# deepinv/deepinv

Hardware: AMD Instinct MI355X
Metric: PnP-PGD slices/sec (50 iters), 2D MRI 8-coil 320x320, 4x radial mask, DRUNet (higher is better)
Workload: dtype f32: fp32 multiplies and accumulation on the fp32 matrix cores (v_mfma_f32_32x32x2_f32); ResBlock convs as Winograd F(4x4,3x3), U = G g G^T formed in fp64 and rounded once; the three 2x2 stride-2 down convolutions (2 % of the FLOPs) as an exact three-part bf16 operand split with six products and fp3

## Files before the change

### deepinv_amd/csrc/drunet_bf16s.hip

```cpp
#include "drunet_common.hpp"

using namespace dinv;
using namespace dinv_drunet;

namespace {

__device__ __forceinline__ unsigned f2bf(float f) {
#ifdef DINV_EMU
    unsigned u = __float_as_uint(f);
    if ((u & 0x7fffffffu) > 0x7f800000u) return (u >> 16) | 0x40u;
    u += 0x7fffu + ((u >> 16) & 1u);
    return u >> 16;
#else
    return (unsigned)__builtin_bit_cast(unsigned short, (__bf16)f);
#endif
}
__device__ __forceinline__ float bf2f(unsigned h) { return __uint_as_float(h << 16); }

__device__ __forceinline__ void split8(const float4& a, const float4& b, uint4& hi, uint4& lo) {
    const float v[8] = {a.x, a.y, a.z, a.w, b.x, b.y, b.z, b.w};
    unsigned h[8], l[8];
#pragma unroll
    for (int e = 0; e < 8; ++e) {
        h[e] = f2bf(v[e]);
        l[e] = f2bf(v[e] - bf2f(h[e]));
    }
    hi = make_uint4(h[0] | (h[1] << 16), h[2] | (h[3] << 16), h[4] | (h[5] << 16), h[6] | (h[7] << 16));
    lo = make_uint4(l[0] | (l[1] << 16), l[2] | (l[3] << 16), l[4] | (l[5] << 16), l[6] | (l[7] << 16));
}

__device__ __forceinline__ void split8x3(const float4& a, const float4& b, uint4& hi, uint4& mi, uint4& lo) {
    const float v[8] = {a.x, a.y, a.z, a.w, b.x, b.y, b.z, b.w};
    unsigned h[8], m[8], l[8];
#pragma unroll
    for (int e = 0; e < 8; ++e) {
        h[e] = f2bf(v[e]);
        const float r1 = v[e] - bf2f(h[e]);
        m[e] = f2bf(r1);
        l[e] = f2bf(r1 - bf2f(m[e]));
    }
    hi = make_uint4(h[0] | (h[1] << 16), h[2] | (h[3] << 16), h[4] | (h[5] << 16), h[6] | (h[7] << 16));
    mi = make_uint4(m[0] | (m[1] << 16), m[2] | (m[3] << 16), m[4] | (m[5] << 16), m[6] | (m[7] << 16));
    lo = make_uint4(l[0] | (l[1] << 16), l[2] | (l[3] << 16), l[4] | (l[5] << 16), l[6] | (l[7] << 16));
}

#ifdef DINV_EMU
__device__ __forceinline__ f32x16 mfma_bf16(const uint4& a, const uint4& b, const f32x16& c) {
    emu_bf16x8 av, bv;
    std::memcpy(&av, &a, 16);
    std::memcpy(&bv, &b, 16);
    return emu_mfma_f32_32x32x16_bf16(av, bv, c);
}
#else
typedef __bf16 bf16x8 __attribute__((ext_vector_type(8)));
__device__ __forceinline__ f32x16 mfma_bf16(const uint4& a, const uint4& b, const f32x16& c) {
    return __builtin_amdgcn_mfma_f32_32x32x16_bf16(__builtin_bit_cast(bf16x8, a), __builtin_bit_cast(bf16x8, b), c, 0, 0, 0);
}
#endif

struct DownSArgs {
    Geom gi, go;
    const float* x;
    const uint4* w;
    float* y;
    int32_t cin, cout;
    int64_t ntiles, per_xcd;
    DepthMap dm;
};

template <bool ACC, int NPL>
__global__ __launch_bounds__(256) void down2x2_bf16s_kernel(DownSArgs a) {
    constexpr int WU = NPL * 128;
    constexpr int WPT = (WU + 255) / 256;
    __shared__ uint4 wl[2][WU];
    const int tid = threadIdx.x, lane = tid & 63, wv = tid >> 6;
    const int l31 = lane & 31, lhi = lane >> 5;
    const int64_t logical = (int64_t)(blockIdx.x & 7) * a.per_xcd + (blockIdx.x >> 3);
    if (logical >= a.ntiles) return;
    const int nct = a.cout / 64;
    const int64_t q0 = (logical / nct) * 256 + wv * 64;
    const int co0 = (int)(logical % nct) * 64;
    int64_t ioff[2];
    bool in[2];
#pragma unroll
    for (int n = 0; n < 2; ++n) {
        const int64_t q = q0 + n * 32 + l31;
        in[n] = interior(a.go, q);
        ioff[n] = a.gi.sl;
        if (in[n]) {
            const int64_t b = q / a.go.plane;
            const int64_t bi = depth_pair(a.dm, b);
            if (bi < 0) in[n] = false;
            else {
                const int qi = (int)(q - b * a.go.plane);
                const int R = qi / a.go.wp, C = qi - R * a.go.wp;
                ioff[n] = a.gi.sl + bi * a.gi.plane + (int64_t)(2 * (R - 1) + 1) * a.gi.wp + (2 * (C - 1) + 1);
            }
        }
    }
    f32x16 acc[2][2];
#pragma unroll
    for (int m = 0; m < 2; ++m)
#pragma unroll
        for (int n = 0; n < 2; ++n)
#pragma unroll
            for (int r = 0; r < 16; ++r) acc[m][n][r] = 0.f;
    const int S = a.cin / 16, nsteps = 4 * S;
    float4 ba[2], bb[2];
    uint4 wreg[WPT];
    auto issue = [&](int g) {
        const int tap = g / S, s = g - tap * S;
        const int64_t toff = (int64_t)(tap >> 1) * a.gi.wp + (tap & 1);
#pragma unroll
        for (int k = 0; k < WPT; ++k) {
            const int u = tid + 256 * k;
            if (u < WU) wreg[k] = a.w[((int64_t)g * (2 * NPL) + (u >> 6)) * a.cout + co0 + (u & 63)];
        }
#pragma unroll
        for (int n = 0; n < 2; ++n) {
            const float* xb = a.x + ((int64_t)(2 * s + lhi) * a.gi.cs + ioff[n] + toff) * 8;
            ba[n] = ld4(xb);
            bb[n] = ld4(xb + 4);
        }
    };
    uint4 Bp[NPL][2];
    auto commit = [&](int stage) {
#pragma unroll
        for (int k = 0; k < WPT; ++k)
            if (tid + 256 * k < WU) wl[stage][tid + 256 * k] = wreg[k];
#pragma unroll
        for (int n = 0; n < 2; ++n) {
            if constexpr (NPL == 2) split8(ba[n], bb[n], Bp[0][n], Bp[1][n]);
            else split8x3(ba[n], bb[n], Bp[0][n], Bp[1][n], Bp[2][n]);
        }
    };
    issue(0);
    commit(0);
    if (nsteps > 1) issue(1);
    __syncthreads();
    constexpr int NPROD = NPL == 2 ? 3 : 6;
    constexpr int PA[6] = {0, 1, 0, 0, 1, 0}, PB2[3] = {1, 0, 0};
    constexpr int QA[6] = {1, 0, 2, 0, 1, 0}, QB[6] = {1, 2, 0, 1, 0, 0};
    for (int g = 0; g < nsteps; ++g) {
        const uint4* ws = wl[g & 1];
        uint4 A[NPL][2];
#pragma unroll
        for (int pl = 0; pl < NPL; ++pl)
#pragma unroll
            for (int m = 0; m < 2; ++m) A[pl][m] = ws[pl * 128 + lhi * 64 + m * 32 + l31];
#pragma unroll
        for (int e = 0; e < NPROD; ++e) {
            const int pa = NPL == 2 ? PA[e] : QA[e], pb = NPL == 2 ? PB2[e] : QB[e];
#pragma unroll
            for (int m = 0; m < 2; ++m)
#pragma unroll
                for (int n = 0; n < 2; ++n) acc[m][n] = mfma_bf16(A[pa][m], Bp[pb][n], acc[m][n]);
        }
        if (g + 1 < nsteps) {
            commit((g + 1) & 1);
            if (g + 2 < nsteps) issue(g + 2);
        }
        lds_barrier();
    }
#pragma unroll
    for (int n = 0; n < 2; ++n) {
        const int64_t q = q0 + n * 32 + l31;
        if (q >= a.go.np) continue;
        store_tile<2, false, ACC ? 1 : 0>(acc, n, a.go.sl + q, in[n], co0 / 8, a.cout / 8, a.go.cs, lhi, a.y, ACC ? a.y : nullptr,
                                          nullptr);
    }
}

struct UpSArgs {
    Geom gi, go;
    const float* x;
    const float* x2;
    const uint4* w;
    float* y;
    int32_t cin, cout;
    DepthMap dm;
};

#ifdef DINV_EMU
#define DINV_BF16S_UP_ATTR
#else
#define DINV_BF16S_UP_ATTR __attribute__((amdgpu_waves_per_eu(2, 2)))
#endif
template <bool SKIP>
__global__ __launch_bounds__(256) DINV_BF16S_UP_ATTR void up2x2_bf16s_kernel(UpSArgs a) {
    __shared__ uint4 wl[2][1024];
    const int tid = threadIdx.x, lane = tid & 63, wv = tid >> 6;
    const int l31 = lane & 31, lhi = lane >> 5;
    const int tp = wv & 1, pg = wv >> 1;
    const int co0 = blockIdx.y * 64;
    const int64_t p0 = (int64_t)blockIdx.x * 128 + pg * 64;
    int64_t ioff[2], ooff[2];
    bool in[2];
#pragma unroll
    for (int n = 0; n < 2; ++n) {
        const int64_t p = p0 + n * 32 + l31;
        in[n] = interior(a.gi, p);
        ioff[n] = a.gi.sl + (in[n] ? p : 0);
        ooff[n] = 0;
        if (in[n]) {
            const int64_t b = p / a.gi.plane;
            const int64_t bo = depth_pair(a.dm, b);
            if (bo < 0) in[n] = false;
            else {
                const int pi = (int)(p - b * a.gi.plane);
                const int r = pi / a.gi.wp, c = pi - r * a.gi.wp;
                ooff[n] = a.go.sl + bo * a.go.plane + (int64_t)(2 * (r - 1) + 1 + tp) * a.go.wp + (2 * (c - 1) + 1);
            }
        }
    }
    f32x16 acc[2][2][2];
#pragma unroll
    for (int t = 0; t < 2; ++t)
#pragma unroll
        for (int m = 0; m < 2; ++m)
#pragma unroll
            for (int n = 0; n < 2; ++n)
#pragma unroll
                for (int r = 0; r < 16; ++r) acc[t][m][n][r] = 0.f;
    const int S = a.cin / 16;
    float4 ba[2], bb[2];
    uint4 wreg[4];
    auto issue = [&](int s) {
#pragma unroll
        for (int k = 0; k < 4; ++k) {
            const int u = tid + 256 * k;
            wreg[k] = a.w[((int64_t)s * 16 + (u >> 6)) * a.cout + co0 + (u & 63)];
        }
#pragma unroll
        for (int n = 0; n < 2; ++n) {
            const int64_t o = ((int64_t)(2 * s + lhi) * a.gi.cs + ioff[n]) * 8;
            ba[n] = ld4(a.x + o);
            bb[n] = ld4(a.x + o + 4);
            if (SKIP) {
                ba[n] = add4(ba[n], ld4(a.x2 + o));
                bb[n] = add4(bb[n], ld4(a.x2 + o + 4));
            }
        }
    };
    auto commit = [&](int stage, uint4 (&Bh)[2], uint4 (&Bl)[2]) {
#pragma unroll
        for (int k = 0; k < 4; ++k) wl[stage][tid + 256 * k] = wreg[k];
        split8(ba[0], bb[0], Bh[0], Bl[0]);
        split8(ba[1], bb[1], Bh[1], Bl[1]);
    };
    uint4 Bh[2], Bl[2];
    issue(0);
    commit(0, Bh, Bl);
    if (S > 1) issue(1);
    __syncthreads();
    for (int s = 0; s < S; ++s) {
        const uint4* ws = wl[s & 1] + (tp * 2) * 256;
#pragma unroll
        for (int t = 0; t < 2; ++t) {
            uint4 A[2][2];
#pragma unroll
            for (int pl = 0; pl < 2; ++pl)
#pragma unroll
                for (int m = 0; m < 2; ++m) A[pl][m] = ws[t * 256 + pl * 128 + lhi * 64 + m * 32 + l31];
#pragma unroll
            for (int e = 0; e < 3; ++e) {
                const int pa = e == 1 ? 1 : 0;
#pragma unroll
                for (int m = 0; m < 2; ++m)
#pragma unroll
                    for (int n = 0; n < 2; ++n) acc[t][m][n] = mfma_bf16(A[pa][m], e == 0 ? Bl[n] : Bh[n], acc[t][m][n]);
            }
        }
        if (s + 1 < S) {
            commit((s + 1) & 1, Bh, Bl);
            if (s + 2 < S) issue(s + 2);
        }
        lds_barrier();
    }
#pragma unroll
    for (int n = 0; n < 2; ++n) {
        if (!in[n]) continue;
#pragma unroll
        for (int t = 0; t < 2; ++t)
#pragma unroll
            for (int m = 0; m < 2; ++m)
#pragma unroll
                for (int rj = 0; rj < 4; ++rj) {
                    const float4 v = make_float4(acc[t][m][n][4 * rj], acc[t][m][n][4 * rj + 1], acc[t][m][n][4 * rj + 2],
                                                 acc[t][m][n][4 * rj + 3]);
                    st4(a.y + ((int64_t)(co0 / 8 + m * 4 + rj) * a.go.cs + ooff[n] + t) * 8 + 4 * lhi, v);
                }
    }
}

}

static int down2x2_bf16s_launch(const dinv_act_geom* gin, const dinv_act_geom* gout, const float* x, const void* w_split,
                                int32_t cin, int32_t cout, float* y, DepthMap dm, int accumulate, dinv_stream_t stream,
                                int planes = 2) {
    if (int e = check_geom(gin)) return e;
    if (int e = check_geom(gout)) return e;
    DINV_REQUIRE(x && w_split && y, "null tensor pointer");
    DINV_REQUIRE(gin->height == 2 * gout->height && gin->width == 2 * gout->width, "down2x2 geometry mismatch");
    if (dm.dep_s == 0) DINV_REQUIRE(gin->batch == gout->batch, "down2x2 geometry mismatch");
    else
        DINV_REQUIRE(dm.dep_s >= 3 && dm.dep_l == 2 * (dm.dep_s - 2) + 2 && gout->batch % dm.dep_s == 0 &&
                     gin->batch / dm.dep_l == gout->batch / dm.dep_s && gin->batch % dm.dep_l == 0 && (dm.dz == 0 || dm.dz == 1),
                     "down2x2: bad depth pairing (%d, %d, %d)", dm.dep_s, dm.dep_l, dm.dz);
    DINV_REQUIRE(cin >= 16 && cin % 16 == 0 && cout % 64 == 0, "bf16-split down2x2 needs cin %% 16 == 0 and cout %% 64 == 0 (got %d,%d)", cin, cout);
    DownSArgs a{make_geom(*gin), make_geom(*gout), x, reinterpret_cast<const uint4*>(w_split), y, cin, cout, 0, 0, dm};
    a.ntiles = ceil_div(gout->np, 256) * (cout / 64);
    a.per_xcd = ceil_div(a.ntiles, 8);
    const dim3 grid((unsigned)(a.per_xcd * 8));
    hipStream_t st = reinterpret_cast<hipStream_t>(stream);
    if (planes == 3) hipLaunchKernelGGL((down2x2_bf16s_kernel<false, 3>), grid, dim3(256), 0, st, a);
    else if (accumulate) hipLaunchKernelGGL((down2x2_bf16s_kernel<true, 2>), grid, dim3(256), 0, st, a);
    else hipLaunchKernelGGL((down2x2_bf16s_kernel<false, 2>), grid, dim3(256), 0, st, a);
    DINV_CHECK_LAUNCH();
    return 0;
}

extern "C" int dinv_conv_down2x2_bf16s(const dinv_act_geom* gin, const dinv_act_geom* gout, const float* x,
                                       const void* w_split, int32_t cin, int32_t cout, float* y, dinv_stream_t stream) {
    return down2x2_bf16s_launch(gin, gout, x, w_split, cin, cout, y, DepthMap{0, 0, 0}, 0, stream);
}

extern "C" int dinv_conv_down2x2_bf16x3(const dinv_act_geom* gin, const dinv_act_geom* gout, const float* x,
                                        const void* w_split3, int32_t cin, int32_t cout, float* y, dinv_stream_t stream) {
    return down2x2_bf16s_launch(gin, gout, x, w_split3, cin, cout, y, DepthMap{0, 0, 0}, 0, stream, 3);
}

extern "C" int dinv_conv_down2x2_bf16s_3d(const dinv_act_geom* gin, const dinv_act_geom* gout, const float* x,
                                          const void* w_split, int32_t cin, int32_t cout, float* y, int32_t depth_out,
                                          int32_t dz, int32_t accumulate, dinv_stream_t stream) {
    DINV_REQUIRE(depth_out >= 1, "bad depth %d", depth_out);
    return down2x2_bf16s_launch(gin, gout, x, w_split, cin, cout, y, DepthMap{depth_out + 2, 2 * depth_out + 2, dz}, accumulate, stream);
}

static int up2x2_bf16s_launch(const dinv_act_geom* gin, const dinv_act_geom* gout, const float* x, const float* x2,
                              const void* w_split, int32_t cin, int32_t cout, float* y, DepthMap dm, dinv_stream_t stream) {
    if (int e = check_geom(gin)) return e;
    if (int e = check_geom(gout)) return e;
    DINV_REQUIRE(x && w_split && y, "null tensor pointer");
    DINV_REQUIRE(gout->height == 2 * gin->height && gout->width == 2 * gin->width, "up2x2 geometry mismatch");
    if (dm.dep_s == 0) DINV_REQUIRE(gin->batch == gout->batch, "up2x2 geometry mismatch");
    else
        DINV_REQUIRE(dm.dep_s >= 3 && dm.dep_l == 2 * (dm.dep_s - 2) + 2 && gin->batch % dm.dep_s == 0 &&
                     gout->batch % dm.dep_l == 0 && gout->batch / dm.dep_l == gin->batch / dm.dep_s && (dm.dz == 0 || dm.dz == 1),
                     "up2x2: bad depth pairing (%d, %d, %d)", dm.dep_s, dm.dep_l, dm.dz);
    DINV_REQUIRE(cin >= 16 && cin % 16 == 0 && cout % 64 == 0, "bf16-split up2x2 needs cin %% 16 == 0 and cout %% 64 == 0 (got %d,%d)", cin, cout);
    UpSArgs a{make_geom(*gin), make_geom(*gout), x, x2, reinterpret_cast<const uint4*>(w_split), y, cin, cout, dm};
    const dim3 grid((unsigned)ceil_div(gin->np, 128), (unsigned)(cout / 64));
    hipStream_t st = reinterpret_cast<hipStream_t>(stream);
    if (x2) hipLaunchKernelGGL(up2x2_bf16s_kernel<true>, grid, dim3(256), 0, st, a);
    else hipLaunchKernelGGL(up2x2_bf16s_kernel<false>, grid, dim3(256), 0, st, a);
    DINV_CHECK_LAUNCH();
    return 0;
}

extern "C" int dinv_conv_up2x2_bf16s(const dinv_act_geom* gin, const dinv_act_geom* gout, const float* x, const float* x2,
                                     const void* w_split, int32_t cin, int32_t cout, float* y, dinv_stream_t stream) {
    return up2x2_bf16s_launch(gin, gout, x, x2, w_split, cin, cout, y, DepthMap{0, 0, 0}, stream);
}

extern "C" int dinv_conv_up2x2_bf16s_3d(const dinv_act_geom* gin, const dinv_act_geom* gout, const float* x, const float* x2,
                                        const void* w_split, int32_t cin, int32_t cout, float* y, int32_t depth_in, int32_t dz,
                                        dinv_stream_t stream) {
    DINV_REQUIRE(depth_in >= 1, "bad depth %d", depth_in);
    return up2x2_bf16s_launch(gin, gout, x, x2, w_split, cin, cout, y, DepthMap{depth_in + 2, 2 * depth_in + 2, dz}, stream);
}
```

Baseline: 16.22.

## Double-register pipeline and reorder K loop in bf16-split down conv

Rewrites the down2x2 bf16-split kernel's main loop. It now keeps two register sets of prefetched activations and weights and issues the next global load before the MFMAs, unrolling by two. The K iteration is reordered to row-tap-major with pairs of horizontal taps merged into a single channel block (via lhi), which changes the weight packing index. It aims to hide global load latency better at the cost of more registers, and it relies on a matching weight layout on the host side.

Measured after the change: 16.32 (median of 6 runs). Within noise of the previous version (+0.6%).

```diff
diff --git a/deepinv_amd/csrc/drunet_bf16s.hip b/deepinv_amd/csrc/drunet_bf16s.hip
--- a/deepinv_amd/csrc/drunet_bf16s.hip
+++ b/deepinv_amd/csrc/drunet_bf16s.hip
@@ -71,7 +71,6 @@
 template <bool ACC, int NPL>
 __global__ __launch_bounds__(256) void down2x2_bf16s_kernel(DownSArgs a) {
     constexpr int WU = NPL * 128;
-    constexpr int WPT = (WU + 255) / 256;
     __shared__ uint4 wl[2][WU];
     const int tid = threadIdx.x, lane = tid & 63, wv = tid >> 6;
     const int l31 = lane & 31, lhi = lane >> 5;
@@ -105,44 +104,38 @@
         for (int n = 0; n < 2; ++n)
 #pragma unroll
             for (int r = 0; r < 16; ++r) acc[m][n][r] = 0.f;
-    const int S = a.cin / 16, nsteps = 4 * S;
-    float4 ba[2], bb[2];
-    uint4 wreg[WPT];
-    auto issue = [&](int g) {
-        const int tap = g / S, s = g - tap * S;
-        const int64_t toff = (int64_t)(tap >> 1) * a.gi.wp + (tap & 1);
-#pragma unroll
-        for (int k = 0; k < WPT; ++k) {
-            const int u = tid + 256 * k;
-            if (u < WU) wreg[k] = a.w[((int64_t)g * (2 * NPL) + (u >> 6)) * a.cout + co0 + (u & 63)];
-        }
-#pragma unroll
-        for (int n = 0; n < 2; ++n) {
-            const float* xb = a.x + ((int64_t)(2 * s + lhi) * a.gi.cs + ioff[n] + toff) * 8;
-            ba[n] = ld4(xb);
-            bb[n] = ld4(xb + 4);
-        }
+    const int S = a.cin / 16, ncb = 2 * S, nsteps = 2 * ncb;
+    const int pd0 = tid >> 6, pd1 = 4 + ((tid & 127) >> 6);
+    auto wunit = [&](int dy, int cb, int pd) {
+        return ((((int64_t)(2 * dy + (pd & 1)) * S + (cb >> 1)) * NPL + (pd >> 1)) * 2 + (cb & 1)) * a.cout + co0 + (tid & 63);
     };
+    float4 xa00, xb00, xa01, xb01, xa10, xb10, xa11, xb11;
+    uint4 wq00, wq01, wq10, wq11;
+    wq01 = wq11 = make_uint4(0, 0, 0, 0);
+#define DINV_ISSUE(G, XA0, XB0, XA1, XB1, W0, W1)                                                                       \
+    {                                                                                                                   \
+        const int dy_ = (G) / ncb, cb_ = (G) - dy_ * ncb;                                                               \
+        W0 = a.w[wunit(dy_, cb_, pd0)];                                                                                 \
+        if constexpr (NPL == 3) W1 = a.w[wunit(dy_, cb_, pd1)];                                                         \
+        const float* x0_ = a.x + ((int64_t)cb_ * a.gi.cs + ioff[0] + (int64_t)dy_ * a.gi.wp + lhi) * 8;                 \
+        const float* x1_ = a.x + ((int64_t)cb_ * a.gi.cs + ioff[1] + (int64_t)dy_ * a.gi.wp + lhi) * 8;                 \
+        XA0 = ld4(x0_); XB0 = ld4(x0_ + 4); XA1 = ld4(x1_); XB1 = ld4(x1_ + 4);                                         \
+    }
     uint4 Bp[NPL][2];
-    auto commit = [&](int stage) {
-#pragma unroll
-        for (int k = 0; k < WPT; ++k)
-            if (tid + 256 * k < WU) wl[stage][tid + 256 * k] = wreg[k];
-#pragma unroll
-        for (int n = 0; n < 2; ++n) {
-            if constexpr (NPL == 2) split8(ba[n], bb[n], Bp[0][n], Bp[1][n]);
-            else split8x3(ba[n], bb[n], Bp[0][n], Bp[1][n], Bp[2][n]);
-        }
-    };
-    issue(0);
-    commit(0);
-    if (nsteps > 1) issue(1);
-    __syncthreads();
+#define DINV_COMMIT(STAGE, XA0, XB0, XA1, XB1, W0, W1)                                                                  \
+    {                                                                                                                   \
+        wl[STAGE][tid] = W0;                                                                                            \
+        if constexpr (NPL == 3) { if (tid < 128) wl[STAGE][256 + tid] = W1; }                                           \
+        if constexpr (NPL == 2) { split8(XA0, XB0, Bp[0][0], Bp[1][0]); split8(XA1, XB1, Bp[0][1], Bp[1][1]); }         \
+        else { split8x3(XA0, XB0, Bp[0][0], Bp[1][0], Bp[2][0]); split8x3(XA1, XB1, Bp[0][1], Bp[1][1], Bp[2][1]); }    \
+    }
+#define DINV_SET0 xa00, xb00, xa01, xb01, wq00, wq01
+#define DINV_SET1 xa10, xb10, xa11, xb11, wq10, wq11
+#define DINV_CALL(M, ...) M(__VA_ARGS__)
     constexpr int NPROD = NPL == 2 ? 3 : 6;
     constexpr int PA[6] = {0, 1, 0, 0, 1, 0}, PB2[3] = {1, 0, 0};
     constexpr int QA[6] = {1, 0, 2, 0, 1, 0}, QB[6] = {1, 2, 0, 1, 0, 0};
-    for (int g = 0; g < nsteps; ++g) {
-        const uint4* ws = wl[g & 1];
+    auto mma = [&](const uint4* ws) {
         uint4 A[NPL][2];
 #pragma unroll
         for (int pl = 0; pl < NPL; ++pl)
@@ -156,12 +149,26 @@
 #pragma unroll
                 for (int n = 0; n < 2; ++n) acc[m][n] = mfma_bf16(A[pa][m], Bp[pb][n], acc[m][n]);
         }
-        if (g + 1 < nsteps) {
-            commit((g + 1) & 1);
-            if (g + 2 < nsteps) issue(g + 2);
-        }
+    };
+    DINV_CALL(DINV_ISSUE, 0, DINV_SET0)
+    DINV_CALL(DINV_COMMIT, 0, DINV_SET0)
+    DINV_CALL(DINV_ISSUE, 1, DINV_SET1)
+    __syncthreads();
+    for (int g = 0; g < nsteps; g += 2) {
+        DINV_CALL(DINV_ISSUE, min(g + 2, nsteps - 1), DINV_SET0)
+        mma(wl[0]);
+        DINV_CALL(DINV_COMMIT, 1, DINV_SET1)
         lds_barrier();
-    }
+        DINV_CALL(DINV_ISSUE, min(g + 3, nsteps - 1), DINV_SET1)
+        mma(wl[1]);
+        if (g + 2 < nsteps) DINV_CALL(DINV_COMMIT, 0, DINV_SET0)
+        lds_barrier();
+    }
+#undef DINV_ISSUE
+#undef DINV_COMMIT
+#undef DINV_SET0
+#undef DINV_SET1
+#undef DINV_CALL
 #pragma unroll
     for (int n = 0; n < 2; ++n) {
         const int64_t q = q0 + n * 32 + l31;
```
